# CDCgov/NowcastAutoGP

Measured on AMD Instinct MI355X. Metric: particle-logml/s (fit+forecast hot path: covariance assembly + Cholesky + logml + predictive per (particle, scenario) item), n=2048 64-particle SMC, higher is better.
Workload: dtype f64

## Files before the change

nowcastautogp_amd/csrc/ngp_api.hip:

```cpp
#include <algorithm>
#include <chrono>
#include <cmath>
#include <condition_variable>
#include <cstdio>
#include <cstdlib>
#include <cstring>
#include <dlfcn.h>
#include <map>
#include <memory>
#include <mutex>
#include <new>
#include <string>
#include <vector>

#include "ngp_internal.h"

using namespace ngp;

#define HIPCHK(expr)                                                     \
    do {                                                                 \
        hipError_t e__ = (expr);                                         \
        if (e__ != hipSuccess) return (ngp_status)(e__ > 0 ? e__ : 999); \
    } while (0)

namespace {
class PinnedPool {
    std::mutex mu;
    std::multimap<size_t, void *> free_;
    std::map<void *, std::pair<size_t, bool>> live_;
    size_t cached_ = 0;
    static constexpr size_t MAX_CACHED = (size_t)256 << 20, MAX_PINNED_BLOCK = (size_t)8 << 20;
    static size_t size_class(size_t n) {
        size_t c = 4096;
        while (c < n) c <<= 1;
        return c;
    }
public:
    void *take(size_t n) {
        const size_t c = size_class(n);
        {
            std::lock_guard<std::mutex> lk(mu);
            auto it = free_.find(c);
            if (it != free_.end()) {
                void *p = it->second;
                free_.erase(it);
                cached_ -= c;
                return p;
            }
        }
        void *p = nullptr;
        bool pinned = c <= MAX_PINNED_BLOCK &&
                      hipHostMalloc(&p, c, hipHostMallocPortable | hipHostMallocMapped) == hipSuccess && p;
        if (!pinned) {
            (void)hipGetLastError();
            p = std::malloc(c);
            if (!p) throw std::bad_alloc();
        }
        std::lock_guard<std::mutex> lk(mu);
        live_[p] = {c, pinned};
        return p;
    }
    bool is_pinned(const void *p) {
        std::lock_guard<std::mutex> lk(mu);
        auto it = live_.find(const_cast<void *>(p));
        return it != live_.end() && it->second.second;
    }
    void give(void *p) {
        std::lock_guard<std::mutex> lk(mu);
        auto it = live_.find(p);
        if (it == live_.end()) return;
        const size_t c = it->second.first;
        if (c <= MAX_PINNED_BLOCK && (c <= ((size_t)256 << 10) || cached_ + c <= MAX_CACHED)) {
            free_.emplace(c, p);
            cached_ += c;
            return;
        }
        const bool pinned = it->second.second;
        live_.erase(it);
        if (pinned) (void)hipHostFree(p);
        else std::free(p);
    }
    ~PinnedPool() {
        for (auto &kv : free_) {
// ... 552 lines not shown
    if (!c || !out) return NGP_ERR_ARG;
    std::lock_guard<std::mutex> lk(c->mu);
    *out = c->prof;
    return NGP_OK;
}

struct ngp_job {
    ngp_ctx *ctx = nullptr;
    JobGeom g{};
    int n = 0;
    bool ran = false;
    DevProgram *progs = nullptr;
    double *t0 = nullptr, *taux = nullptr, *y0 = nullptr, *ya = nullptr;
    double *logdet = nullptr, *G = nullptr, *work = nullptr, *zbuf = nullptr;
    int32_t *info = nullptr, *qpts = nullptr;
    double *logml_base = nullptr, *logml_full = nullptr, *mu = nullptr, *sigma = nullptr;
    int64_t work_stride = 0;
    std::vector<void *> owned;
    PinVec<unsigned char> h_in, h_out;
    size_t out_off[5] = {}, out_bytes = 0;
    bool zeroed = false, copy_in_flight = false;
    bool out_fetched = false;
    ngp_spec spec{};
    std::vector<int32_t> fill_chain, fill_other, fill_single;
    int32_t *fill_chain_d = nullptr, *fill_other_d = nullptr, *fill_single_d = nullptr;
    std::vector<int32_t> refine_steps;
    std::vector<double> refine_delta, frac32;
};

namespace {

struct EventTimer {
    struct Rec { int cls; hipEvent_t a, b; double flops, bytes; };
    std::vector<Rec> recs;
    bool on;
    hipStream_t s;
    EventTimer(bool on_, hipStream_t s_) : on(on_), s(s_) {}
    ~EventTimer() {
        for (auto &r : recs) {
            (void)hipEventDestroy(r.a);
            (void)hipEventDestroy(r.b);
        }
    }
    template <class F> void run(int cls, double flops, double bytes, F &&f,
                                hipStream_t on_stream = nullptr) {
        if (!on) { f(); return; }
        hipStream_t es = on_stream ? on_stream : s;
        Rec r{cls, nullptr, nullptr, flops, bytes};
        (void)hipEventCreate(&r.a);
        (void)hipEventCreate(&r.b);
        (void)hipEventRecord(r.a, es);
        f();
        (void)hipEventRecord(r.b, es);
        recs.push_back(r);
    }
    void resolve(ngp_profile &p) {
        for (auto &r : recs) {
            float ms = 0.f;
            if (hipEventElapsedTime(&ms, r.a, r.b) == hipSuccess) {
                p.ms[r.cls] += ms;
                p.launches[r.cls] += 1;
                p.flops[r.cls] += r.flops;
                p.bytes[r.cls] += r.bytes;
            }
            (void)hipEventDestroy(r.a);
            (void)hipEventDestroy(r.b);
        }
        recs.clear();
    }
};


struct Lane {
    hipStream_t main, side;
    hipEvent_t fork, join;
    ngp_ctx *ctx;
};
inline Lane lane_of(ngp_ctx *c) { return Lane{c->stream, c->side, c->ev_fork, c->ev_join, c}; }

constexpr size_t MAX_CHUNK_ITEMS = 65535;
inline bool item_too_large(int64_t item_stride) { return item_stride * 8 > (int64_t)0x7fffffff; }
constexpr int MIXED_REORDER = 16;
constexpr int AHEAD_EARLY_MAX_ITEMS = 512;
constexpr int TWO_LANE_MIN_ITEMS = 64, TWO_LANE_MIN_NB = 24;
void factor_chunk(const Lane &ln, const JobGeom &g, const ChunkPtrs &p_in, int bc, EventTimer &tm,
                  size_t dinv_step = 0, const DevSpec *sp = nullptr, int32_t *order_buf = nullptr,
                  unsigned *order_prev = nullptr, bool half = false) {
    ChunkPtrs p0 = p_in;
    const bool mixed = sp != nullptr && p0.L32 != nullptr;
    hipStream_t s = ln.main;
    SmallPlan spl;
    if (!mixed && dinv_step == 0 && small_job(g, bc, &spl)) {
        const double nn = 16.0 * spl.nbe;
        tm.run(13, bc * small_flops(g, spl), bc * 8.0 * (nn * nn * (spl.ident ? 1.5 : 1.0) + 2.0 * g.naux * nn),
               [&] { launch_chol_small(g, p0, bc, spl, s); });
        return;
    }
    if (!half && bc <= AHEAD_EARLY_MAX_ITEMS && !mixed && !g.aux_identity && g.nb0 >= 8 && !g.invariant &&
        ln.ctx->splitk_reserve(bc) == NGP_OK)
        p0.splitk_part = ln.ctx->splitk_part;
    const int nl = ngp_ctx::MAX_LANES;
    if (!half && !mixed && nl >= 2 && bc >= TWO_LANE_MIN_ITEMS && bc <= AHEAD_EARLY_MAX_ITEMS &&
        g.nb0 >= TWO_LANE_MIN_NB && ln.main == ln.ctx->stream && ln.ctx->make_lanes(nl)) {
        ngp_ctx *c = ln.ctx;
        (void)hipEventRecord(c->ev_lane_go, s);
        std::vector<EventTimer> tms;
        tms.reserve((size_t)nl);
        int h0 = 0;
        for (int i = 0; i < nl; ++i) {
            const int h1 = (int)((long)bc * (i + 1) / nl);
            ChunkPtrs pi = p0;
            pi.L += (size_t)h0 * g.item_stride;
            pi.dinv += (size_t)h0 * NB * NB;
            pi.progs += h0;
            pi.logdet += h0;
            pi.info += h0;
            if (pi.tab) pi.tab += (size_t)h0 * g.maxstat * g.R;
            pi.n_fill_single = (int32_t)((long)p0.n_fill_single * (h1 - h0) / bc);
            if (pi.splitk_part) pi.splitk_part += (size_t)h0 * SPLITK_SLOTS * 4 * 64 * 64;
            if (i == 0) {
                factor_chunk(ln, g, pi, h1 - h0, tm, dinv_step, sp, order_buf, order_prev, true);
            } else {
                const Lane li{c->lane_main[i], c->lane_side[i], c->lane_fork[i], c->lane_join[i], c};
                tms.emplace_back(tm.on, li.main);
                (void)hipStreamWaitEvent(li.main, c->ev_lane_go, 0);
                factor_chunk(li, g, pi, h1 - h0, tms.back(), dinv_step, sp, order_buf, order_prev, true);
                (void)hipEventRecord(c->lane_done[i], li.main);
            }
            h0 = h1;
        }
        for (int i = 1; i < nl; ++i) (void)hipStreamWaitEvent(s, c->lane_done[i], 0);
        for (auto &t : tms) {
            tm.recs.insert(tm.recs.end(), t.recs.begin(), t.recs.end());
            t.recs.clear();
        }
        return;
    }
    const double nrows_aux = (double)g.naux;
    const double lazy_frac =
        (g.toep && p0.n_fill_single > 0 && !mixed) ? std::min(1.0, (double)p0.n_fill_single / bc) : 0.0;
    bool ahead_pending = false;
    const int o = (g.nb0 >= 3 && (g.nb0 & 1)) ? 1 : 0;
    for (int jj = 0; jj < g.nb0; ++jj) {
        const bool fat = jj >= o && ((jj - o) % 2 == 0) && (jj + 1 < g.nb0);
        const bool thin = jj >= o && ((jj - o) % 2 == 1);
        const int mode = fat ? COL_FAT : (thin ? COL_THIN : COL_FULL);
        const int ahead = (fat && jj + 2 < g.nb0) ? 1 : 0;
        const int k0_col = thin ? (jj - 1) * NB : 0;
        const int k0_diag = thin ? (jj - 1) * NB : (jj - o >= 2 ? (jj - 2) * NB : 0);
        const double k = (double)jj * NB;
        const double kd = k - k0_diag;
        ChunkPtrs p = p0;
        p.dinv = p0.dinv + (size_t)jj * dinv_step;
        if (ahead_pending && ((jj - o) % 2 == 0)) {
            (void)hipStreamWaitEvent(s, ln.join, 0);
            ahead_pending = false;
        }
        const bool ahead_early = bc <= AHEAD_EARLY_MAX_ITEMS;
        auto launch_ahead = [&] {
            (void)hipEventRecord(ln.fork, s);
            (void)hipStreamWaitEvent(ln.side, ln.fork, 0);
            tm.run(8, bc * (double)NB * NB * k, bc * 8.0 * NB * k,
                   [&] { launch_diag_ahead(g, p0, bc, jj, ln.side); }, ln.side);
            (void)hipEventRecord(ln.join, ln.side);
            ahead_pending = true;
        };
        if (ahead && jj > 0 && ahead_early) launch_ahead();
        tm.run(1, bc * ((double)NB * NB * kd + (double)NB * NB * NB / 3.0),
               bc * 8.0 * (NB * kd + 2.0 * NB * NB),
               [&] { launch_chol_diag(g, p, bc, jj, k0_diag, s); });
        double rows = (double)(g.n0 - (jj + 1) * NB) + nrows_aux;
        const double kc = k - k0_col;
        double rows_kc = rows * kc;
        if (g.aux_identity) {
            rows = (double)(g.n0 - (jj + 1) * NB) + (double)(g.naux - g.n0);
            rows_kc = rows * kc;
            for (int a = 0; a <= jj && a < g.nb0; ++a) {
                rows += NB;
                rows_kc += NB * std::max(0.0, k - std::max((double)k0_col, (double)a * NB));
            }
        }
        double fl = 2.0 * NB * rows_kc + rows * (double)NB * NB;
        double by = 8.0 * (rows_kc + NB * kc + 2.0 * rows * NB);
        if (fat) {
            fl += 2.0 * NB * rows_kc;
            by += 8.0 * (NB * k + 2.0 * rows * NB);
        }
        if (lazy_frac > 0.0 && (fat || (mode == COL_FULL && jj == 0))) {
            const double rm = (double)(g.n0 - (jj + 1) * NB);
            by -= lazy_frac * 8.0 * NB * (rm + (fat ? std::max(0.0, rm - NB) : 0.0));
        }
        tm.run(fat ? (mixed ? 9 : (g.aux_identity ? 12 : 0)) : 6, bc * fl, bc * by,
               [&] { launch_chol_col(g, p, bc, jj, mode, k0_col, s, sp); });
        if (mixed && fat && order_buf && jj >= 8 && jj % MIXED_REORDER == 8) {
            if (launch_mixed_order(p0, order_prev, order_buf, bc, s)) p0.order = order_buf;
        }
        if (ahead && jj > 0 && !ahead_early) launch_ahead();
    }
    if (ahead_pending) {
        (void)hipStreamWaitEvent(s, ln.join, 0);
        ahead_pending = false;
    }
}

constexpr size_t STAGE_KEEP_BYTES = (size_t)4 << 20, FETCH_PACKED_BYTES = (size_t)1 << 20;

template <class T> ngp_status job_alloc(ngp_job *j, T **p, size_t count) {
    void *v = nullptr;
    ngp_status st = j->ctx->alloc(&v, count * sizeof(T));
    if (st) return st;
    j->owned.push_back(v);
    *p = (T *)v;
    return NGP_OK;
}

ngp_status stage_general(ngp_ctx *c, int P, const ngp_kernel *kernels, int n, const double *t,
                         const double *y, int64_t ldy, int d, const double *t_add, int D,
                         const double *y_add, int64_t ld_yadd_item, int m, const double *t_new,
                         int noise_on_new, ngp_job **out, const double *const *yrows = nullptr) {
    if (!c || !out || !kernels || P <= 0 || n < 0 || d < 0 || m < 0 || D <= 0) return NGP_ERR_ARG;
    if (n + d <= 0) return NGP_ERR_ARG;
    if ((n > 0 && (!t || (!y && !yrows))) || (d > 0 && (!t_add || !y_add)) || (m > 0 && !t_new))
        return NGP_ERR_ARG;
    *out = nullptr;
    auto yrow = [&](int b) { return yrows ? yrows[b] : y + (int64_t)b * ldy; };
    std::vector<DevProgram> hp((size_t)P);
    int maxstat = 0, maxcp = 0;
    for (int i = 0; i < P; ++i) {
        int ns = 0, nc = 0, nt = 0;
        ngp_status st = compile_program(&kernels[i], &hp[(size_t)i], nullptr, &ns, &nc, &nt);
        if (st) return st;
        maxstat = std::max(maxstat, nt);
        maxcp = std::max(maxcp, nc);
    }
    JobGeom g{};
    g.B = P;
    g.n0 = (n / NB) * NB;
    g.nb0 = g.n0 / NB;
    g.tail = n - g.n0;
    g.da = g.tail + d;
    g.d = d;
    g.m = m;
    g.naux = g.da + m + 1;
    if (g.naux > NGP_MAX_AUX) return NGP_ERR_TOO_LARGE;
    g.naux_pad = (g.naux + NB - 1) / NB * NB;
    g.D = D;
    g.noise_on_new = noise_on_new ? 1 : 0;
    g.y_shared = (ldy == 0 && !yrows) ? 1 : 0;
    g.ld = g.n0;
    g.item_stride = (int64_t)(g.n0 + g.naux_pad) * g.n0;
    if (item_too_large(g.item_stride)) return NGP_ERR_TOO_LARGE;
    g.npts = g.n0 + g.da + m;
    g.n_real = g.n0;
    g.aux_identity = 0;
    g.maxstat = std::max(maxstat, 1);
    g.maxcp = std::max(maxcp, 1);
    std::vector<int32_t> h_q;
    int32_t toep_stride = 0;
    if (g.n0 > 0) {
        std::vector<double> allt((size_t)g.npts);
        for (int i = 0; i < n; ++i) allt[(size_t)i] = t[i];
        for (int a = 0; a < d; ++a) allt[(size_t)(n + a)] = t_add[a];
        for (int i = 0; i < m; ++i) allt[(size_t)(n + d + i)] = t_new[i];
        double hh = 0.0;
        int R = 0;
        if (detect_lattice(allt, &hh, &h_q, &R)) {
            g.lattice = 1;
            g.h = hh;
            g.R = R;
            if (g.nb0 >= 2) {
                const long st0 = (long)h_q[1] - (long)h_q[0];
                bool reg = st0 != 0;
                for (int i = 2; i < g.n0 && reg; ++i)
                    reg = (long)h_q[(size_t)i] - (long)h_q[(size_t)i - 1] == st0;
                if (reg) toep_stride = (int32_t)std::labs(st0);
// ... 147 lines not shown
                   });
    };
    backward(0);
    std::vector<double> dprev((size_t)bc, 1.0), dboth(2 * (size_t)bc, 0.0);
    std::vector<int32_t> active((size_t)bc);
    for (int i = 0; i < bc; ++i) { steps[i] = 0; delta_out[i] = 0.0; active[(size_t)i] = i; }
    for (int it = 1;; ++it) {
        tm.run(10, na * 2.0 * naux * n0 * n0, na * 8.0 * 3.0 * naux * n0,
               [&] { launch_kapply(g, pf, rb.A, rb.X, rb.R, na, sp, s); });
        tm.run(10, na * 4.0 * naux * naux * n0, na * 8.0 * 3.0 * naux * n0, [&] {
            launch_refine_gram(g, rb.A, rb.X, rb.R, rb.S, rb.T, rb.U, Gchunk, rb.delta, na,
                               pf.items, s);
        });
        HIPCHK(hipMemcpyAsync(dboth.data(), rb.delta, sizeof(double) * 2 * (size_t)bc,
                              hipMemcpyDeviceToHost, s));
        HIPCHK(hipStreamSynchronize(s));
        std::vector<int32_t> still;
        for (int i : active) {
            const double d = dboth[2 * (size_t)i];
            double rho = dboth[2 * (size_t)i + 1];
            if (it > 1) rho = std::max(rho, d / dprev[(size_t)i]);
            const double est = d * std::min(rho, 1.0);
            steps[i] = it;
            delta_out[i] = d;
            dprev[(size_t)i] = d;
            if (!(est <= spec.refine_tol)) still.push_back(i);
        }
        active.swap(still);
        if (active.empty() || it >= spec.refine_max) break;
        na = (int)active.size();
        HIPCHK(hipMemcpy(rb.items, active.data(), 4 * (size_t)na, hipMemcpyHostToDevice));
        pf.items = rb.items;
        for (int i : active)
            HIPCHK(hipMemcpyAsync(p.L + (size_t)i * g.item_stride + (size_t)g.n0 * g.ld,
                                  rb.R + (size_t)i * g.naux_pad * g.n0,
                                  (size_t)g.naux_pad * g.n0 * 8, hipMemcpyDeviceToDevice, s));
        for (int jj = 0; jj < g.nb0; ++jj) {
            ChunkPtrs pj = pf;
            pj.dinv = p.dinv + (size_t)jj * mstep;
            tm.run(10, na * naux * (double)NB * NB, na * 8.0 * 3.0 * naux * NB,
                   [&] { launch_chol_col(g, pj, na, jj, COL_AUX, jj * NB, s); });
            tm.run(10, na * naux * 2.0 * NB * (double)(g.n0 - (jj + 1) * NB),
                   na * 8.0 * (g.n0 - (jj + 1) * NB) * (2.0 * naux + NB),
                   [&] { launch_aux_update(g, pj, na, jj, s); });
        }
        backward(1);
    }
    for (int i : active) not_refined->push_back(i);
    return NGP_OK;
}

}

extern "C" ngp_status ngp_job_run(ngp_job *j) {
    if (!j) return NGP_ERR_ARG;
    ngp_ctx *c = j->ctx;
    std::lock_guard<std::mutex> lk(c->mu);
    HIPCHK(hipSetDevice(c->device));
    const JobGeom &g = j->g;
    hipStream_t s = c->stream;
    const DevSpec sp = dev_spec(j->spec);
    EventTimer tm(c->profiling, s);
    if (!j->zeroed && !(g.n0 > 0 && small_job(g, g.B) && j->spec.precision != NGP_PREC_MIXED)) {
        HIPCHK(hipMemsetAsync(j->logdet, 0, sizeof(double) * (size_t)g.B, s));
        HIPCHK(hipMemsetAsync(j->info, 0, sizeof(int32_t) * (size_t)g.B, s));
    }
    j->zeroed = false;
    const bool mixed = j->spec.precision == NGP_PREC_MIXED && g.nb0 >= 2 && g.nb0 <= 129 &&
                       !g.aux_identity;
    const bool refine = mixed && j->spec.refine_max > 0;
    j->refine_steps.assign((size_t)g.B, 0);
    j->refine_delta.assign((size_t)g.B, 0.0);
    j->frac32.assign((size_t)g.B, 0.0);
    void *Lbuf = nullptr, *dinv = nullptr, *tab = nullptr, *sig = nullptr;
    void *L32 = nullptr, *tmx = nullptr, *cnt = nullptr, *order_buf = nullptr, *order_prev = nullptr;
    RefineBufs rb;
    bool single_chunk = false;
    if (g.n0 > 0) {
        const size_t tab_bytes = g.lattice ? sizeof(double) * (size_t)g.maxstat * g.R : 0;
        const size_t sig_bytes = g.lattice ? sizeof(double) * (size_t)g.maxcp * g.npts : 0;
        const size_t l_bytes = (size_t)g.item_stride * sizeof(double);
        const size_t nbt = (size_t)g.nb0 + (size_t)g.naux_pad / NB;
        const size_t aux_bytes = sizeof(double) * (size_t)g.naux_pad * g.n0;
        size_t item_bytes = l_bytes + tab_bytes + sig_bytes + sizeof(double) * NB * NB;
        if (mixed)
            item_bytes += l_bytes / 2 + 4 * nbt * g.nb0 + aux_bytes + 16 +
                          (refine ? sizeof(double) * NB * NB * (size_t)g.nb0 + 2 * aux_bytes +
                                        16 * (size_t)g.naux * g.naux + 8 * (size_t)g.naux + 20
                                  : 0);
        if ((size_t)g.B * item_bytes > c->mem_cap) c->refresh_mem_cap();
        const size_t bc_max = std::min<size_t>(
            std::min<size_t>((size_t)g.B, MAX_CHUNK_ITEMS), std::max<size_t>(1, c->mem_cap / item_bytes));
        size_t nchunks = ((size_t)g.B + bc_max - 1) / bc_max;
        int Bc = 0;
        size_t mstep = 0;
        ngp_status st = NGP_OK;
        auto take_all = [&](WsPlan &dalloc) -> ngp_status {
            ngp_status st = dalloc(&Lbuf, l_bytes * (size_t)Bc);
            if (!st) st = dalloc(&dinv, sizeof(double) * (size_t)Bc * NB * NB * (refine ? g.nb0 : 1));
            if (!st && g.lattice) st = dalloc(&tab, tab_bytes * (size_t)Bc);
            if (!st && g.lattice) st = dalloc(&sig, sig_bytes * (size_t)Bc);
            if (!st && mixed) {
                st = dalloc(&L32, (l_bytes / 2) * (size_t)Bc);
                if (!st) st = dalloc(&tmx, 4 * nbt * g.nb0 * (size_t)Bc);
                if (!st) st = dalloc(&cnt, 8 * (size_t)Bc);
                if (!st) st = dalloc(&order_buf, 4 * (size_t)Bc);
                if (!st) st = dalloc(&order_prev, 4 * (size_t)Bc);
                if (!st) st = dalloc((void **)&rb.X, aux_bytes * (size_t)Bc);
            }
            if (!st && refine) {
                st = dalloc((void **)&rb.A, aux_bytes * (size_t)Bc);
                if (!st) st = dalloc((void **)&rb.R, aux_bytes * (size_t)Bc);
                if (!st) st = dalloc((void **)&rb.S, 8 * (size_t)g.naux * g.naux * Bc);
                if (!st) st = dalloc((void **)&rb.T, 8 * (size_t)g.naux * g.naux * Bc);
                if (!st) st = dalloc((void **)&rb.U, 8 * (size_t)g.naux * Bc);
                if (!st) st = dalloc((void **)&rb.delta, 16 * (size_t)Bc);
                if (!st) st = dalloc((void **)&rb.items, 4 * (size_t)Bc);
            }
            return st;
        };
        for (;; nchunks *= 2) {
            Bc = (int)(((size_t)g.B + nchunks - 1) / nchunks);
            mstep = refine ? (size_t)Bc * NB * NB : 0;
            WsPlan measure{c, true}, take{c, false};
            (void)take_all(measure);
            st = c->ws_reserve(measure.total);
            if (!st) st = take_all(take);
            if (st != NGP_ERR_TOO_LARGE || Bc <= 1) break;
        }
        single_chunk = Bc >= g.B;
        if (st) return st;
        const Lane ln = lane_of(c);
        const double nrows_aux = (double)g.naux;
        for (int b0 = 0; b0 < g.B; b0 += Bc) {
            const int bc = std::min(Bc, g.B - b0);
            ChunkPtrs p{};
            p.L = (double *)Lbuf;
            p.dinv = (double *)dinv;
            p.progs = j->progs + b0;
            p.t0 = j->t0;
            p.taux = j->taux;
            p.y0 = j->y0 + (g.y_shared ? 0 : (int64_t)b0 * g.n0);
            p.logdet = j->logdet + b0;
            p.info = j->info + b0;
            p.tab = (double *)tab;
            p.sig = (double *)sig;
            p.qpts = j->qpts;
            if (j->fill_other_d) {
                auto range = [&](const std::vector<int32_t> &v, const int32_t *dev,
                                 const int32_t **ptr, int32_t *cnt) {
                    const auto lo = std::lower_bound(v.begin(), v.end(), b0);
                    const auto hi = std::lower_bound(v.begin(), v.end(), b0 + bc);
                    *ptr = dev + (lo - v.begin());
                    *cnt = (int32_t)(hi - lo);
                };
                range(j->fill_chain, j->fill_chain_d, &p.fill_chain, &p.n_fill_chain);
                range(j->fill_other, j->fill_other_d, &p.fill_other, &p.n_fill_other);
                range(j->fill_single, j->fill_single_d, &p.fill_single, &p.n_fill_single);
                p.fill_base = b0;
            }
            if (mixed) {
                p.L32 = (float *)L32;
                p.tmax = (float *)tmx;
                p.mixcnt = (unsigned *)cnt;
                p.auxX = rb.X;
                HIPCHK(hipMemsetAsync(cnt, 0, 8 * (size_t)bc, s));
            }
            if (g.lattice)
                tm.run(4, 0.0, 0.0, [&] { launch_tables(g, p, bc, sp, s); });
            const double fill_elems =
                (double)bc * ((double)g.n0 * (g.n0 + NB) / 2.0 + nrows_aux * g.n0) -
                (g.toep ? (double)p.n_fill_single * ((double)g.n0 * (g.n0 - NB) / 2.0) : 0.0);
            tm.run(4, 0.0, 8.0 * fill_elems, [&] { launch_fill(g, p, bc, sp, s); });
            if (mixed) HIPCHK(hipMemsetAsync(order_prev, 0, 4 * (size_t)bc, s));
            double *Gchunk = j->G + (int64_t)b0 * g.naux * g.naux;
            const bool gram_inside = !mixed && mstep == 0 && small_job(g, bc);
            if (gram_inside) p.G = Gchunk;
            factor_chunk(ln, g, p, bc, tm, mstep, mixed ? &sp : nullptr, (int32_t *)order_buf,
                         (unsigned *)order_prev);
            if (!gram_inside)
                tm.run(2, bc * nrows_aux * nrows_aux * g.n0, bc * 8.0 * nrows_aux * g.n0,
                       [&] { launch_gram(g, (const double *)Lbuf, Gchunk, bc, s); });
            if (mixed) {
                std::vector<unsigned> hc(2 * (size_t)bc);
                HIPCHK(hipMemcpyAsync(hc.data(), cnt, 8 * (size_t)bc, hipMemcpyDeviceToHost, s));
                std::vector<int> bad;
                if (refine) {
                    ngp_status rs = refine_chunk(c, g, p, rb, Gchunk, bc, mstep, j->spec, sp, tm,
                                                 j->refine_steps.data() + b0,
                                                 j->refine_delta.data() + b0, &bad);
                    if (rs) { tm.resolve(c->prof); return rs; }
                } else {
                    HIPCHK(hipStreamSynchronize(s));
                }
                for (int i = 0; i < bc; ++i) {
                    const double a = hc[2 * (size_t)i], b = hc[2 * (size_t)i + 1];
                    j->frac32[(size_t)(b0 + i)] = (a + b) > 0.0 ? a / (a + b) : 0.0;
                }
                if (!bad.empty()) {
                    std::vector<int32_t> hi((size_t)bc);
                    HIPCHK(hipMemcpy(hi.data(), p.info, 4 * (size_t)bc, hipMemcpyDeviceToHost));
                    for (int i : bad)
                        if (hi[(size_t)i] == 0) hi[(size_t)i] = NGP_INFO_NOT_REFINED;
                    HIPCHK(hipMemcpy(p.info, hi.data(), 4 * (size_t)bc, hipMemcpyHostToDevice));
                }
            }
        }
    }
    EpiPtrs e{};
    e.progs = j->progs;
    e.taux = j->taux;
    e.G = j->G;
    e.ya = j->ya;
    e.logdet = j->logdet;
    e.info = j->info;
    e.work = j->work;
    e.zbuf = j->zbuf;
    e.logml_base = j->logml_base;
    e.logml_full = j->logml_full;
    e.mu = j->mu;
    e.sigma = j->sigma;
// ... 1923 lines not shown
```

nowcastautogp_amd/csrc/ngp_col_kernels.h:

```cpp
#pragma once
#include <algorithm>

#include "ngp_mfma.h"

namespace ngp {

struct NoProbe {
    __device__ __forceinline__ void mark(int) {}
    template <class T>
    __device__ __forceinline__ void mark_after(int, T) {}
    __device__ __forceinline__ void drain() {}
    __device__ __forceinline__ void emit_diag(int, int, int) {}
    __device__ __forceinline__ void emit_col(int, int, int, int, int, int, bool) {}
    __device__ __forceinline__ void begin(int, int, int) {}
    __device__ __forceinline__ void sweep(int) {}
};

__device__ __forceinline__ void sqrt_and_rcp(double a, double &d, double &r) {
    double y = __builtin_amdgcn_rsq(a);
    const double h = 0.5 * a;
    y = y * fma(-h * y, y, 1.5);
    y = y * fma(-h * y, y, 1.5);
    d = a * y;
    d = fma(fma(-d, d, a), 0.5 * y, d);
    r = fma(fma(-d, y, 1.0), y, y);
}

__device__ __forceinline__ int tri(int r, int c) { return ((r * (r + 1)) >> 1) + c; }
constexpr int TRI = NB * (NB + 1) / 2;

template <class Probe = NoProbe>
__global__ __launch_bounds__(256, 4) void chol_diag_kernel(JobGeom g, ChunkPtrs p, int j, int k0) {
    __shared__ double Mt[TRI];
    __shared__ double Lt[TRI];
    __shared__ double pan[NB][4];
    __shared__ double dblk[16];
    __shared__ double dinvd[4];
    __shared__ double rdg[NB];
    __shared__ double logs[NB];
    __shared__ double Ts[TB][TB + 1];
    __shared__ int bad;
    const int item = blockIdx.x;
    const int tid = threadIdx.x, lane = tid & 63;
    const int wave = __builtin_amdgcn_readfirstlane(tid >> 6);
    const long ld = g.ld;
    double *Lit = p.L + (long)item * g.item_stride;
    double *Lj = Lit + (long)j * NB * ld;
    const int kmax = j * NB;
    const int r16 = lane & 15, q = lane >> 4;
    const int wr = wave >> 1, wc = wave & 1;
    Probe probe;
    probe.mark_after(0, lane);

    if (tid == 0) bad = 0;

    if (!(wr == 0 && wc == 1)) {
        double acc4[2][2][4];
#pragma unroll
        for (int a = 0; a < 2; ++a)
#pragma unroll
            for (int b = 0; b < 2; ++b)
#pragma unroll
                for (int r = 0; r < 4; ++r) acc4[a][b][r] = 0.0;
        const double *pa = Lj + (long)(32 * wr + r16) * ld + 2 * q;
        const double *pb = Lj + (long)(32 * wc + r16) * ld + 2 * q;
        double kt[2][2][4];
#pragma unroll
        for (int mt = 0; mt < 2; ++mt)
#pragma unroll
            for (int nt = 0; nt < 2; ++nt)
#pragma unroll
                for (int s = 0; s < 4; ++s)
                    kt[mt][nt][s] = Lj[(long)(32 * wr + 16 * mt + q + 4 * s) * ld + kmax +
                                       32 * wc + 16 * nt + r16];
        for (int kc = k0; kc < kmax; kc += 16) {
            double a[2][4], b[2][4];
#pragma unroll
            for (int u = 0; u < 2; ++u) {
                const f64x2 alo = *reinterpret_cast<const f64x2 *>(pa + (long)u * 16 * ld + kc);
                const f64x2 ahi = *reinterpret_cast<const f64x2 *>(pa + (long)u * 16 * ld + kc + 8);
                const f64x2 blo = *reinterpret_cast<const f64x2 *>(pb + (long)u * 16 * ld + kc);
                const f64x2 bhi = *reinterpret_cast<const f64x2 *>(pb + (long)u * 16 * ld + kc + 8);
                a[u][0] = alo.x; a[u][1] = alo.y; a[u][2] = ahi.x; a[u][3] = ahi.y;
                b[u][0] = blo.x; b[u][1] = blo.y; b[u][2] = bhi.x; b[u][3] = bhi.y;
            }
#pragma unroll
            for (int s = 0; s < 4; ++s)
#pragma unroll
                for (int nt = 0; nt < 2; ++nt) {
                    const Rot4 br = rot4(b[nt][s]);
#pragma unroll
                    for (int mt = 0; mt < 2; ++mt) mfma16_as_4(acc4[mt][nt], a[mt][s], br);
                }
        }
        f64x4 acc[2][2];
#pragma unroll
        for (int a = 0; a < 2; ++a)
#pragma unroll
            for (int b = 0; b < 2; ++b) acc[a][b] = to_d16(acc4[a][b]);
#pragma unroll
        for (int mt = 0; mt < 2; ++mt)
#pragma unroll
            for (int nt = 0; nt < 2; ++nt)
#pragma unroll
                for (int s = 0; s < 4; ++s) {
                    const int M = 32 * wr + 16 * mt + q + 4 * s, N = 32 * wc + 16 * nt + r16;
                    if (M >= N) Mt[tri(M, N)] = kt[mt][nt][s] - acc[mt][nt][s];
                }
    }
    __syncthreads();
    probe.mark_after(1, lane);

    const int bi = tid >> 4, bj = tid & 15;
    {
        double a[4][4];
#pragma unroll
        for (int r = 0; r < 4; ++r)
#pragma unroll
            for (int c = 0; c < 4; ++c) {
                const int R = 4 * bi + r, C = 4 * bj + c;
                a[r][c] = (R >= C) ? Mt[tri(R, C)] : 0.0;
            }
        for (int kb = 0; kb < NB / 4; ++kb) {
            if (bi == kb && bj == kb) {
                double dks[4];
#pragma unroll
                for (int kc = 0; kc < 4; ++kc) {
                    const double akk = a[kc][kc];
                    double dk, inv;
                    sqrt_and_rcp(akk, dk, inv);
                    if (!(akk > 0.0) && bad == 0) bad = 4 * kb + kc + 1;
                    dks[kc] = dk;
                    dinvd[kc] = inv;
                    rdg[4 * kb + kc] = inv;
// ... 39 lines not shown
            __syncthreads();
            if (bj > kb && bi >= bj) {
                double li[4][4], lj[4][4];
#pragma unroll
                for (int r = 0; r < 4; ++r)
#pragma unroll
                    for (int pp = 0; pp < 4; ++pp) {
                        li[r][pp] = pan[4 * bi + r][pp];
                        lj[r][pp] = pan[4 * bj + r][pp];
                    }
#pragma unroll
                for (int pp = 0; pp < 4; ++pp)
#pragma unroll
                    for (int r = 0; r < 4; ++r)
#pragma unroll
                        for (int c = 0; c < 4; ++c) a[r][c] -= li[r][pp] * lj[c][pp];
            }
        }
#pragma unroll
        for (int r = 0; r < 4; ++r) {
            const int R = 4 * bi + r;
            f64x2 lo, hi;
            lo.x = (R >= 4 * bj) ? a[r][0] : 0.0;
            lo.y = (R >= 4 * bj + 1) ? a[r][1] : 0.0;
            hi.x = (R >= 4 * bj + 2) ? a[r][2] : 0.0;
            hi.y = (R >= 4 * bj + 3) ? a[r][3] : 0.0;
            double *dst = Lj + (long)R * ld + kmax + 4 * bj;
            *reinterpret_cast<f64x2 *>(dst) = lo;
            *reinterpret_cast<f64x2 *>(dst + 2) = hi;
#pragma unroll
            for (int c = 0; c < 4; ++c)
                if (R >= 4 * bj + c) Lt[tri(R, 4 * bj + c)] = a[r][c];
        }
    }
    __syncthreads();
    probe.mark_after(2, lane);
    if (tid < NB) logs[tid] = log(Lt[tri(tid, tid)]);

    if (tid < NB) {
        const int b = tid >> 4, c = tid & 15;
        double x[TB];
#pragma unroll
        for (int i = 0; i < TB; ++i) {
            double sum = (i == c) ? 1.0 : 0.0;
            int off = tri(TB * b + i, TB * b);
            if (i > 0) asm volatile("" : "+v"(off) : "v"(x[i - 1]));
            const double *lrow = &Lt[off];
#pragma unroll
            for (int pp = 0; pp < i; ++pp) sum -= lrow[pp] * x[pp];
            x[i] = sum * rdg[TB * b + i];
        }
#pragma unroll
        for (int i = 0; i < TB; ++i)
            if (i >= c) Mt[tri(TB * b + i, TB * b + c)] = x[i];
    }
    __syncthreads();
    probe.mark_after(3, lane);
    {
        const int ra = tid >> 4, cb = tid & 15;
        for (int dist = 1; dist < NB / TB; ++dist)
            for (int ct = dist; ct < NB / TB; ++ct) {
                const int jt = ct - dist;
                double t = 0.0;
                for (int kt = jt; kt < ct; ++kt)
#pragma unroll
                    for (int pp = 0; pp < TB; ++pp) {
                        const double mv = Mt[tri(TB * kt + pp, TB * jt + cb)];
                        t += Lt[tri(TB * ct + ra, TB * kt + pp)] * ((kt > jt || pp >= cb) ? mv : 0.0);
                    }
                Ts[ra][cb] = t;
                __syncthreads();
                double mv = 0.0;
#pragma unroll
                for (int pp = 0; pp < TB; ++pp) {
                    const double md = Mt[tri(TB * ct + ra, TB * ct + pp)];
                    mv -= ((pp <= ra) ? md : 0.0) * Ts[pp][cb];
                }
                Mt[tri(TB * ct + ra, TB * jt + cb)] = mv;
                __syncthreads();
            }
    }
    probe.mark_after(4, lane);
    {
        double *dv = p.dinv + (long)item * (NB * NB);
        for (int e = tid; e < NB * NB; e += 256) {
            const int strip = e >> 6, l = e & 63;
            const int cb4 = strip >> 2, jt = strip & 3;
            const int R = 4 * cb4 + (l & 3), C = 16 * jt + 4 * ((l >> 2) & 3) + (l >> 4);
            dv[e] = (R >= C) ? Mt[tri(R, C)] : 0.0;
        }
    }
    if (tid == 0) {
        double s = 0.0;
        for (int k = 0; k < NB; ++k) s += logs[k];
        p.logdet[item] += s;
        if (bad && p.info[item] == 0) p.info[item] = kmax + bad;
    }
    probe.mark_after(5, lane);
    probe.emit_diag(j, tid, item);
}

template <int NF>
struct Frag8 {
    f64x2 v[NF];
};
template <int NF>
__device__ __forceinline__ void load_frag8(Frag8<NF> &f, const double *p, long ld) {
#pragma unroll
    for (int u = 0; u < NF; ++u) f.v[u] = *reinterpret_cast<const f64x2 *>(p + (long)u * 16 * ld);
}
template <int NA>
__device__ __forceinline__ void mfma_frag8(double (&acc)[NA][4][4], const Frag8<NA> &a,
                                           const Frag8<4> &b) {
#pragma unroll
    for (int it = 0; it < 4; ++it) {
        const Rot4 br = rot4(b.v[it].x);
#pragma unroll
        for (int jt = 0; jt < NA; ++jt) mfma16_as_4(acc[jt][it], a.v[jt].x, br);
    }
#pragma unroll
    for (int it = 0; it < 4; ++it) {
        const Rot4 br = rot4(b.v[it].y);
#pragma unroll
        for (int jt = 0; jt < NA; ++jt) mfma16_as_4(acc[jt][it], a.v[jt].y, br);
    }
}

template <int NA>
__device__ __forceinline__ void gemm_rows(double (&acc)[NA][4][4], const double *pa,
                                          const double *pb, long ld, int k0, int k1) {
    if (k1 <= k0) return;
    Frag8<NA> a0, a1;
    Frag8<4> b0, b1;
    load_frag8(a0, pa + k0, ld);
    load_frag8(b0, pb + k0, ld);
    for (int kc = k0; kc < k1; kc += 16) {
        load_frag8(a1, pa + kc + 8, ld);
        load_frag8(b1, pb + kc + 8, ld);
        mfma_frag8(acc, a0, b0);
        if (kc + 16 < k1) {
            load_frag8(a0, pa + kc + 16, ld);
            load_frag8(b0, pb + kc + 16, ld);
        }
        mfma_frag8(acc, a1, b1);
    }
}

constexpr int EPI_PITCH = 66;
constexpr int EPI_M_BYTES = NB * NB * 8;
constexpr int EPI_WAVE_BYTES = 16 * EPI_PITCH * 8;
constexpr int EPI_LDS_BYTES = EPI_M_BYTES + 4 * EPI_WAVE_BYTES;

__device__ __forceinline__ void stage_mstrips(double *lds_m, const double *mstrips, int tid) {
#pragma unroll
    for (int i = 0; i < 8; ++i) {
        const int idx = tid + 256 * i;
        reinterpret_cast<f64x2 *>(lds_m)[idx] = reinterpret_cast<const f64x2 *>(mstrips)[idx];
    }
}

template <bool SHADOW = false, bool SYNTH = false, class Probe = NoProbe, bool KROWS = false>
__device__ __forceinline__ void solve_and_store_lds(const double (*acc4)[4][4], double *Lr,
                                                    const double *lds_m, long ld, int kmax,
                                                    int lane, double *buf, Probe &probe,
                                                    float *Lr32 = nullptr,
                                                    float *tmax_out = nullptr, int synth = 0,
                                                    const double *ksl = nullptr, int nit = 4) {
    double amax = 0.0;
    const int n16 = lane & 15, isub = lane >> 4;
    const int jj0 = 4 * (n16 >> 2) + isub;
    const double *ksl0 = ksl ? ksl + 15 - jj0 : nullptr;
    f64x2 kvr[8];
    double kvp[4][4];
    const int hrow = lane >> 5, c2 = 2 * (lane & 31);
    bool from_rows = KROWS && ksl0 == nullptr;
    if constexpr (SYNTH) from_rows = from_rows && synth == 0;
    auto k_elems = [&](int it, double (&kv)[4][4]) {
        if (ksl0) {
#pragma unroll
            for (int jt = 0; jt < 4; ++jt)
#pragma unroll
                for (int r = 0; r < 4; ++r)
// ... 752 lines not shown
#pragma unroll
                for (int jl = 0; jl < 2; ++jl)
#pragma unroll
                    for (int it = 0; it < 4; ++it)
#pragma unroll
                        for (int r = 0; r < 4; ++r)
                            acc4[2 * a + jl][it][r] =
                                t64[(16 * jl + jj0) * P64 + 16 * it + ((r16 + 4 * r) & 15)];
                __syncthreads();
            }
        }
        if (n64 > 0) {
            unsigned long long lo = m64lo, hi = m64hi;
            const int nch = 4 * n64;
            int kt_cur = pop(lo, hi), sub = 1;
            stage(0, kt_cur * NB);
            __syncthreads();
            for (int c = 0; c < nch; ++c) {
                const int cur = c & 1;
                if (c + 1 < nch) {
                    if (sub == 4) {
                        kt_cur = pop(lo, hi);
                        sub = 0;
                    }
                    stage(cur ^ 1, kt_cur * NB + LDS_KC * sub);
                    ++sub;
                }
                mult_chunk_pipelined<2 * BLKB>(acc4, smem + cur * STAGE, a_addr, b_addr);
                __syncthreads();
            }
        }
    }
    if constexpr (SPLITK == 1) {
        double *mine = p.splitk_part +
                       ((((long)slot * SPLITK_SLOTS + (long)grp * st.splits + piece) * 4 + wave) *
                        (64 * 64)) + lane;
#pragma unroll
        for (int jt = 0; jt < 4; ++jt)
#pragma unroll
            for (int it = 0; it < 4; ++it)
#pragma unroll
                for (int r = 0; r < 4; ++r) mine[((jt * 4 + it) * 4 + r) * 64] = acc4[jt][it][r];
        return;
    }
    if constexpr (SPLITK == 2) {
        const double *part = p.splitk_part +
                             ((((long)slot * SPLITK_SLOTS + (long)grp * st.splits) * 4 + wave) *
                              (64 * 64)) + lane;
#pragma unroll
        for (int jt = 0; jt < 4; ++jt)
#pragma unroll
            for (int it = 0; it < 4; ++it)
#pragma unroll
                for (int r = 0; r < 4; ++r) acc4[jt][it][r] = part[((jt * 4 + it) * 4 + r) * 64];
        for (int q2 = 1; q2 < st.splits; ++q2) {
            const double *pq = part + (long)q2 * 4 * (64 * 64);
            double v[4][4][4];
#pragma unroll
            for (int jt = 0; jt < 4; ++jt)
#pragma unroll
                for (int it = 0; it < 4; ++it)
#pragma unroll
                    for (int r = 0; r < 4; ++r) v[jt][it][r] = pq[((jt * 4 + it) * 4 + r) * 64];
#pragma unroll
            for (int jt = 0; jt < 4; ++jt)
#pragma unroll
                for (int it = 0; it < 4; ++it)
#pragma unroll
                    for (int r = 0; r < 4; ++r) acc4[jt][it][r] += v[jt][it][r];
        }
    }
    static_assert(EPI_LDS_BYTES + TOEP_LDS_BYTES <= 2 * STAGE,
                  "epilogue LDS must fit the stage buffers");
    probe.mark(3);
    const double *ksl = nullptr;
    if (structured) {
        double *sl = reinterpret_cast<double *>(smem + EPI_LDS_BYTES) + wave * 128;
        struct_slice(sl, g, p, item, (int)tile_row0(tile), col ? kmax + NB : kmax, lane);
        ksl = sl;
    }
    stage_mstrips(reinterpret_cast<double *>(smem), p.dinv + (long)item * (NB * NB), tid);
    __syncthreads();
    probe.mark(4);
    if (!valid) return;

    double *Lr = Lit + tile_row0(tile) * ld;
    if (col) {
        subtract_in_place_rows(Lr, ld, (j + 1) * NB, acc4, lane,
                               reinterpret_cast<double *>(smem + EPI_M_BYTES + wave * EPI_WAVE_BYTES),
                               IDENT && synth != 0, ksl, nit);
    } else if constexpr (MIXED) {
        const int rt = (tile < st.nmain) ? j + 1 + tile : g.nb0 + (tile - st.nmain);
        solve_and_store_lds<true>(
            acc4, Lr, reinterpret_cast<const double *>(smem), ld, kmax, lane,
            reinterpret_cast<double *>(smem + EPI_M_BYTES + wave * EPI_WAVE_BYTES), probe,
            p.L32 + (long)item * g.item_stride + tile_row0(tile) * ld,
            p.tmax + (long)item * (g.nb0 + g.naux_pad / NB) * g.nb0 + tmax_index(g, rt, j));
    } else {
        solve_and_store_lds<false, IDENT>(
            acc4, Lr, reinterpret_cast<const double *>(smem), ld, kmax, lane,
            reinterpret_cast<double *>(smem + EPI_M_BYTES + wave * EPI_WAVE_BYTES), probe, nullptr,
            nullptr, synth, ksl, nit);
    }
    probe.mark(5);
    probe.drain();
    probe.mark(6);
    probe.emit_col(j, lane, wg, wave, item, tile, false);
}

template <class Probe>
void launch_chol_diag_t(const JobGeom &g, const ChunkPtrs &p, int Bc, int j, int k0, hipStream_t s) {
    hipLaunchKernelGGL(chol_diag_kernel<Probe>, dim3(Bc), dim3(256), 0, s, g, p, j, k0);
}

template <class Probe>
void launch_chol_col_t(const JobGeom &g, const ChunkPtrs &p, int Bc, int j, int mode, int k0,
                     hipStream_t s, const DevSpec *sp) {
    ColStep st{};
    const bool mixed = p.L32 != nullptr && sp != nullptr;
    if (mixed) {
        st.c32 = sp->mixed_tau / (64.0 * 5.9604644775390625e-08);
        st.jitter = sp->jitter;
    }
    st.j = j;
    st.k0 = k0;
    st.nmain = (mode == COL_AUX) ? 0 : g.nb0 - 1 - j;
    st.ntiles = st.nmain + g.naux_pad / NB;
    if (st.ntiles <= 0) return;
    const int bpad = (Bc + 7) / 8 * 8;
    const dim3 blk(256);
    st.first_touch = (mode == COL_FAT || (mode == COL_FULL && k0 == 0 && j == 0)) ? 1 : 0;
    if (mode == COL_FAT) {
        st.groups = (st.ntiles + 1) / 2;
        const dim3 grid(st.groups * bpad);
        int splits = 1;
        if (!mixed && !g.aux_identity && p.splitk_part) {
            const int nchunks = j * NB / LDS_KC;
            splits = std::min(std::min(8, SPLITK_SLOTS / std::max(st.groups, 1)),
                              std::min(nchunks / 8, 384 / std::max(st.groups * Bc, 1)));
        }
        st.splits = std::max(splits, 1);
        if (splits >= 2) {
            hipLaunchKernelGGL((chol_col_glds_kernel<false, Probe, false, 1>),
                               dim3(st.groups * splits * bpad), blk, 0, s, g, p, Bc, st);
            hipLaunchKernelGGL((chol_col_glds_kernel<false, Probe, false, 2>), grid, blk, 0, s, g, p,
                               Bc, st);
        } else if (mixed)
            hipLaunchKernelGGL((chol_col_glds_kernel<true, Probe>), grid, blk, 0, s, g, p, Bc, st);
        else if (g.aux_identity)
            hipLaunchKernelGGL((chol_col_glds_kernel<false, Probe, true>), grid, blk, 0, s, g, p, Bc, st);
        else
            hipLaunchKernelGGL((chol_col_glds_kernel<false, Probe>), grid, blk, 0, s, g, p, Bc, st);
    } else if (mode == COL_THIN && k0 == j * NB - NB && j > 0) {
        st.groups = (st.ntiles + 3) / 4;
        const dim3 grid(st.groups * bpad);
        if (mixed)
            hipLaunchKernelGGL((chol_col_thin_kernel<true, Probe>), grid, blk, 0, s, g, p, Bc, st);
        else if (g.aux_identity)
            hipLaunchKernelGGL((chol_col_thin_kernel<false, Probe, true>), grid, blk, 0, s, g, p, Bc, st);
        else
            hipLaunchKernelGGL((chol_col_thin_kernel<false, Probe>), grid, blk, 0, s, g, p, Bc, st);
    } else {
        st.groups = (st.ntiles + 3) / 4;
        const dim3 grid(st.groups * bpad);
        if (mixed)
            hipLaunchKernelGGL(chol_col_kernel<true>, grid, blk, 0, s, g, p, Bc, st);
        else if (g.aux_identity)
            hipLaunchKernelGGL((chol_col_kernel<false, true>), grid, blk, 0, s, g, p, Bc, st);
        else if (g.toep && st.first_touch)
            hipLaunchKernelGGL((chol_col_kernel<false, false, true>), grid, blk, 0, s, g, p, Bc, st);
        else
            hipLaunchKernelGGL(chol_col_kernel<false>, grid, blk, 0, s, g, p, Bc, st);
    }
}

}
```

nowcastautogp_amd/csrc/ngp_internal.h:

```cpp
#pragma once
#include <hip/hip_runtime.h>
#include <stdint.h>

#include <algorithm>

#include "../../include/ngp.h"

namespace ngp {

constexpr int NB = 64;
constexpr int TB = 16;
constexpr int DEV_STACK = 8;
constexpr int SPLITK_SLOTS = 16;

constexpr int OP_CP_SWAPPED = 9;
constexpr int OP_TABLE = 10;
constexpr int RLEAF_TABLE = 1, RLEAF_LINEAR = 2;
constexpr int MAX_TABLES = NGP_MAX_OPS / 2;

struct DevProgram {
    int32_t n_ops;
    int32_t n_params;
    double  noise;
    uint8_t ops[NGP_MAX_OPS];
    uint8_t slot[NGP_MAX_OPS];
    uint8_t first[NGP_MAX_OPS];
    uint8_t poff[NGP_MAX_OPS];
    double  params[NGP_MAX_PARAMS];
    int32_t n_rops, n_tab;
    int32_t rchain, rpad_;
    uint8_t rops[NGP_MAX_OPS];
    uint8_t rslot[NGP_MAX_OPS];
    uint8_t rpoff[NGP_MAX_OPS];
    uint8_t rleaf[NGP_MAX_OPS];
    uint8_t tb_first[MAX_TABLES];
    uint8_t tb_last[MAX_TABLES];
};
static_assert(sizeof(DevProgram) % 8 == 0, "DevProgram is copied as 8-byte words");
__host__ __device__ inline bool prog_single_table(const DevProgram *P) {
    return P->n_rops == 1 && P->rops[0] == OP_TABLE;
}
__host__ __device__ inline int prog_structure(const DevProgram *P) {
    return (P->n_rops == 1 && P->rops[0] == OP_TABLE) ? 1 : 0;
}
struct DevSpec {
    int32_t se_form, periodic_form, cp_form, precision;
    double  jitter;
    double  mixed_tau;
};

struct JobGeom {
    int32_t B;
    int32_t n0;
    int32_t nb0;
    int32_t da;
    int32_t tail;
    int32_t m;
    int32_t naux;
    int32_t naux_pad;
    int32_t D;
    int32_t d;
    int32_t noise_on_new;
    int32_t y_shared;
    int32_t lattice;
    int32_t R;
    int32_t npts;
    int32_t maxstat;
    int32_t maxcp;
    int32_t n_real;
    int32_t aux_identity;
    int32_t maxops;
    int32_t aux_e1;
    int32_t toep;
    int32_t tab_sub;
    int32_t invariant;
    int32_t short_series;
    int32_t pad_;
    double  h;
    int64_t ld;
    int64_t item_stride;
};

struct ChunkPtrs {
    double       *L;
    double       *dinv;
    const DevProgram *progs;
    const DevProgram *progs_src;
    const double *t0;
    const double *taux;
    const double *y0;
    double       *logdet;
    int32_t      *info;
    double       *tab;
    double       *sig;
    const int32_t *qpts;
    double       *dtab;
    float        *L32;
    float        *tmax;
    unsigned     *mixcnt;
    double       *auxX;
    const int32_t *order;
    const int32_t *fill_chain, *fill_other, *fill_single;
    int32_t n_fill_chain, n_fill_other, n_fill_single, fill_base;
    double       *G;
    const int32_t *items;
    double       *splitk_part;
};

struct EpiPtrs {
    const DevProgram *progs;
    const double *taux;
    const double *G;
    const double *ya;
    const double *logdet;
    int32_t      *info;
    double       *work;
    double       *zbuf;
    double       *logml_base;
    double       *logml_full;
    double       *mu;
    double       *sigma;
    int64_t       work_stride;
    const double *tab, *sig;
    const int32_t *qpts;
};

constexpr int SM_WAVES = 8, SM_THREADS = 64 * SM_WAVES;
constexpr int SM_NSLOT = 20;
constexpr int SM_DSTR = 17;
constexpr int SM_MAX_PANEL = 34;
constexpr int SM_MAX_SWEEPS = 4;
constexpr int SM_MAX_ITEMS = 4096;

struct SmallSweep {
    int32_t main;
    int32_t i0, i1, a0, a1;
};
struct SmallPlan {
    int32_t nbe;
    int32_t nsweeps;
    int32_t ident;
    int32_t npanel;
    uint64_t colwave;
    SmallSweep sw[SM_MAX_SWEEPS];
};

constexpr int SM_LDS_FIXED = 8 * (16 * 256 + 16 * 16 * SM_DSTR + 256 + 32);
inline int small_lds_bytes(const SmallPlan &pl) { return SM_LDS_FIXED + pl.npanel * 2048; }

inline bool small_plan(const JobGeom &g, SmallPlan *pl) {
    if (g.n0 <= 0 || g.nb0 > 4 || g.aux_e1 || g.toep) return false;
    const int nb16 = g.n0 / 16, nbe = (g.n_real + 15) / 16;
    if (nbe < 1 || nbe > nb16) return false;
    const int cap_main = (SM_WAVES - 1) * SM_NSLOT, cap_aux = SM_WAVES * SM_NSLOT;
    SmallPlan p{};
    p.nbe = nbe;
    p.ident = g.aux_identity ? 1 : 0;
    int used = nbe * (nbe - 1) / 2;
    if (used > cap_main) return false;
    int ns = 0, npanel = nbe;
    if (g.aux_identity) {
        const int ytile = nb16;
        if (used + nbe > cap_main) return false;
        p.sw[ns++] = SmallSweep{1, 0, 0, ytile, ytile + 1};
        p.sw[ns++] = SmallSweep{2, 0, nbe, 0, 0};
        npanel = std::max(npanel, nbe + 1);
        int load[SM_WAVES] = {};
        for (int j = 0; j < nbe; ++j) {
            int best = 0;
            for (int w = 1; w < SM_WAVES; ++w) {
                const int sb = load[best % 4] + load[best % 4 + 4], sw_ = load[w % 4] + load[w % 4 + 4];
                if (sw_ < sb || (sw_ == sb && load[w] < load[best])) best = w;
            }
            load[best] += (nbe - j) * (nbe - j - 1) / 2 + 1;
            p.colwave |= (uint64_t)best << (4 * j);
        }
    } else {
        const int nba = (g.naux + 15) / 16;
        int a = std::min(nba, (cap_main - used) / nbe);
        a = std::min(a, SM_MAX_PANEL - nbe);
        p.sw[ns++] = SmallSweep{1, 0, 0, 0, a};
        npanel = std::max(npanel, nbe + a);
        while (a < nba) {
            if (ns == SM_MAX_SWEEPS) return false;
            const int b = std::min(nba, a + std::min(cap_aux / nbe, SM_MAX_PANEL - nbe));
            p.sw[ns++] = SmallSweep{0, 0, 0, a, b};
            npanel = std::max(npanel, nbe + b - a);
            a = b;
        }
// ... 81 lines not shown
```

Measured before the change: 17220.

## Fuse next-column diagonal Cholesky into fat column kernel for large batches

For batches larger than the ahead-early threshold, the fat column kernel's group-0 workgroup now factors the next diagonal block (j+1) after finishing its tile, reusing the stage LDS. The separate chol_diag launch for the following thin column is skipped. A second dinv slot is allocated so the next block's inverse does not overwrite the one still being read. This removes one kernel launch and one sync point per column pair, but serialises the diagonal factorization onto the tail of one workgroup per item and adds LDS aliasing and extra workspace.

```diff
diff --git a/nowcastautogp_amd/csrc/ngp_api.hip b/nowcastautogp_amd/csrc/ngp_api.hip
--- a/nowcastautogp_amd/csrc/ngp_api.hip
+++ b/nowcastautogp_amd/csrc/ngp_api.hip
@@ -1,4 +1,5 @@
 #include <algorithm>
+#include <atomic>
 #include <chrono>
 #include <cmath>
 #include <condition_variable>
@@ -717,6 +718,8 @@
 inline bool item_too_large(int64_t item_stride) { return item_stride * 8 > (int64_t)0x7fffffff; }
 constexpr int MIXED_REORDER = 16;
 constexpr int AHEAD_EARLY_MAX_ITEMS = 512;
+static std::atomic<int> g_diag_fuse{1};
+extern "C" void ngp_debug_set_diag_fuse(int on) { g_diag_fuse.store(on); }
 constexpr int TWO_LANE_MIN_ITEMS = 64, TWO_LANE_MIN_NB = 24;
 void factor_chunk(const Lane &ln, const JobGeom &g, const ChunkPtrs &p_in, int bc, EventTimer &tm,
                   size_t dinv_step = 0, const DevSpec *sp = nullptr, int32_t *order_buf = nullptr,
@@ -753,6 +756,7 @@
             if (pi.tab) pi.tab += (size_t)h0 * g.maxstat * g.R;
             pi.n_fill_single = (int32_t)((long)p0.n_fill_single * (h1 - h0) / bc);
             if (pi.splitk_part) pi.splitk_part += (size_t)h0 * SPLITK_SLOTS * 4 * 64 * 64;
+            if (pi.dinv2) pi.dinv2 += (size_t)h0 * NB * NB;
             if (i == 0) {
                 factor_chunk(ln, g, pi, h1 - h0, tm, dinv_step, sp, order_buf, order_prev, true);
             } else {
@@ -775,6 +779,8 @@
     const double lazy_frac =
         (g.toep && p0.n_fill_single > 0 && !mixed) ? std::min(1.0, (double)p0.n_fill_single / bc) : 0.0;
     bool ahead_pending = false;
+    const bool fuse_diag = g_diag_fuse.load(std::memory_order_relaxed) && bc > AHEAD_EARLY_MAX_ITEMS &&
+                           !mixed && !g.aux_identity && !p0.splitk_part && (dinv_step != 0 || p0.dinv2);
     const int o = (g.nb0 >= 3 && (g.nb0 & 1)) ? 1 : 0;
     for (int jj = 0; jj < g.nb0; ++jj) {
         const bool fat = jj >= o && ((jj - o) % 2 == 0) && (jj + 1 < g.nb0);
@@ -787,6 +793,9 @@
         const double kd = k - k0_diag;
         ChunkPtrs p = p0;
         p.dinv = p0.dinv + (size_t)jj * dinv_step;
+        const bool diag_done = fuse_diag && thin;
+        if (diag_done && !dinv_step) p.dinv = p0.dinv2;
+        if (fuse_diag && fat) p.dinv_next = dinv_step ? p0.dinv + (size_t)(jj + 1) * dinv_step : p0.dinv2;
         if (ahead_pending && ((jj - o) % 2 == 0)) {
             (void)hipStreamWaitEvent(s, ln.join, 0);
             ahead_pending = false;
@@ -801,9 +810,10 @@
             ahead_pending = true;
         };
         if (ahead && jj > 0 && ahead_early) launch_ahead();
-        tm.run(1, bc * ((double)NB * NB * kd + (double)NB * NB * NB / 3.0),
-               bc * 8.0 * (NB * kd + 2.0 * NB * NB),
-               [&] { launch_chol_diag(g, p, bc, jj, k0_diag, s); });
+        auto diag_fl = [&](double kd_) { return bc * ((double)NB * NB * kd_ + (double)NB * NB * NB / 3.0); };
+        auto diag_by = [&](double kd_) { return bc * 8.0 * (NB * kd_ + 2.0 * NB * NB); };
+        if (!diag_done)
+            tm.run(1, diag_fl(kd), diag_by(kd), [&] { launch_chol_diag(g, p, bc, jj, k0_diag, s); });
         double rows = (double)(g.n0 - (jj + 1) * NB) + nrows_aux;
         const double kc = k - k0_col;
         double rows_kc = rows * kc;
@@ -825,7 +835,12 @@
             const double rm = (double)(g.n0 - (jj + 1) * NB);
             by -= lazy_frac * 8.0 * NB * (rm + (fat ? std::max(0.0, rm - NB) : 0.0));
         }
-        tm.run(fat ? (mixed ? 9 : (g.aux_identity ? 12 : 0)) : 6, bc * fl, bc * by,
+        double fl_all = bc * fl, by_all = bc * by;
+        if (fuse_diag && fat) {
+            fl_all += diag_fl(NB);
+            by_all += diag_by(NB);
+        }
+        tm.run(fat ? (mixed ? 9 : (g.aux_identity ? 12 : 0)) : 6, fl_all, by_all,
                [&] { launch_chol_col(g, p, bc, jj, mode, k0_col, s, sp); });
         if (mixed && fat && order_buf && jj >= 8 && jj % MIXED_REORDER == 8) {
             if (launch_mixed_order(p0, order_prev, order_buf, bc, s)) p0.order = order_buf;
@@ -1139,7 +1154,8 @@
         const size_t l_bytes = (size_t)g.item_stride * sizeof(double);
         const size_t nbt = (size_t)g.nb0 + (size_t)g.naux_pad / NB;
         const size_t aux_bytes = sizeof(double) * (size_t)g.naux_pad * g.n0;
-        size_t item_bytes = l_bytes + tab_bytes + sig_bytes + sizeof(double) * NB * NB;
+        const size_t mslots = refine ? (size_t)g.nb0 : (mixed ? 1 : 2);
+        size_t item_bytes = l_bytes + tab_bytes + sig_bytes + sizeof(double) * NB * NB * (refine ? 1 : mslots);
         if (mixed)
             item_bytes += l_bytes / 2 + 4 * nbt * g.nb0 + aux_bytes + 16 +
                           (refine ? sizeof(double) * NB * NB * (size_t)g.nb0 + 2 * aux_bytes +
@@ -1154,7 +1170,7 @@
         ngp_status st = NGP_OK;
         auto take_all = [&](WsPlan &dalloc) -> ngp_status {
             ngp_status st = dalloc(&Lbuf, l_bytes * (size_t)Bc);
-            if (!st) st = dalloc(&dinv, sizeof(double) * (size_t)Bc * NB * NB * (refine ? g.nb0 : 1));
+            if (!st) st = dalloc(&dinv, sizeof(double) * (size_t)Bc * NB * NB * mslots);
             if (!st && g.lattice) st = dalloc(&tab, tab_bytes * (size_t)Bc);
             if (!st && g.lattice) st = dalloc(&sig, sig_bytes * (size_t)Bc);
             if (!st && mixed) {
@@ -1194,6 +1210,7 @@
             ChunkPtrs p{};
             p.L = (double *)Lbuf;
             p.dinv = (double *)dinv;
+            if (mslots == 2) p.dinv2 = (double *)dinv + (size_t)Bc * NB * NB;
             p.progs = j->progs + b0;
             p.t0 = j->t0;
             p.taux = j->taux;
diff --git a/nowcastautogp_amd/csrc/ngp_col_kernels.h b/nowcastautogp_amd/csrc/ngp_col_kernels.h
--- a/nowcastautogp_amd/csrc/ngp_col_kernels.h
+++ b/nowcastautogp_amd/csrc/ngp_col_kernels.h
@@ -29,18 +29,30 @@
 __device__ __forceinline__ int tri(int r, int c) { return ((r * (r + 1)) >> 1) + c; }
 constexpr int TRI = NB * (NB + 1) / 2;
 
-template <class Probe = NoProbe>
-__global__ __launch_bounds__(256, 4) void chol_diag_kernel(JobGeom g, ChunkPtrs p, int j, int k0) {
-    __shared__ double Mt[TRI];
-    __shared__ double Lt[TRI];
-    __shared__ double pan[NB][4];
-    __shared__ double dblk[16];
-    __shared__ double dinvd[4];
-    __shared__ double rdg[NB];
-    __shared__ double logs[NB];
-    __shared__ double Ts[TB][TB + 1];
-    __shared__ int bad;
-    const int item = blockIdx.x;
+struct DiagLds {
+    double Mt[TRI];
+    double Lt[TRI];
+    double pan[NB][4];
+    double dblk[16];
+    double dinvd[4];
+    double rdg[NB];
+    double logs[NB];
+    double Ts[TB][TB + 1];
+    int bad;
+};
+
+template <class Probe>
+__device__ __forceinline__ void chol_diag_block(const JobGeom &g, const ChunkPtrs &p, int item, int j,
+                                                int k0, double *dv, DiagLds &sh, Probe &probe) {
+    double(&Mt)[TRI] = sh.Mt;
+    double(&Lt)[TRI] = sh.Lt;
+    double(&pan)[NB][4] = sh.pan;
+    double(&dblk)[16] = sh.dblk;
+    double(&dinvd)[4] = sh.dinvd;
+    double(&rdg)[NB] = sh.rdg;
+    double(&logs)[NB] = sh.logs;
+    double(&Ts)[TB][TB + 1] = sh.Ts;
+    int &bad = sh.bad;
     const int tid = threadIdx.x, lane = tid & 63;
     const int wave = __builtin_amdgcn_readfirstlane(tid >> 6);
     const long ld = g.ld;
@@ -49,7 +61,6 @@
     const int kmax = j * NB;
     const int r16 = lane & 15, q = lane >> 4;
     const int wr = wave >> 1, wc = wave & 1;
-    Probe probe;
     probe.mark_after(0, lane);
 
     if (tid == 0) bad = 0;
@@ -255,7 +266,7 @@
     }
     probe.mark_after(4, lane);
     {
-        double *dv = p.dinv + (long)item * (NB * NB);
+        dv += (long)item * (NB * NB);
         for (int e = tid; e < NB * NB; e += 256) {
             const int strip = e >> 6, l = e & 63;
             const int cb4 = strip >> 2, jt = strip & 3;
@@ -270,7 +281,14 @@
         if (bad && p.info[item] == 0) p.info[item] = kmax + bad;
     }
     probe.mark_after(5, lane);
-    probe.emit_diag(j, tid, item);
+}
+
+template <class Probe = NoProbe>
+__global__ __launch_bounds__(256, 4) void chol_diag_kernel(JobGeom g, ChunkPtrs p, int j, int k0) {
+    __shared__ DiagLds sh;
+    Probe probe;
+    chol_diag_block(g, p, (int)blockIdx.x, j, k0, p.dinv, sh, probe);
+    probe.emit_diag(j, threadIdx.x, blockIdx.x);
 }
 
 template <int NF>
@@ -1189,10 +1207,13 @@
     stage_mstrips(reinterpret_cast<double *>(smem), p.dinv + (long)item * (NB * NB), tid);
     __syncthreads();
     probe.mark(4);
-    if (!valid) return;
+    bool fuse_diag = false;
+    if constexpr (!MIXED && !IDENT && SPLITK == 0) fuse_diag = p.dinv_next != nullptr && grp == 0;
+    if (!valid && !fuse_diag) return;
 
     double *Lr = Lit + tile_row0(tile) * ld;
-    if (col) {
+    if (!valid) {
+    } else if (col) {
         subtract_in_place_rows(Lr, ld, (j + 1) * NB, acc4, lane,
                                reinterpret_cast<double *>(smem + EPI_M_BYTES + wave * EPI_WAVE_BYTES),
                                IDENT && synth != 0, ksl, nit);
@@ -1213,6 +1234,14 @@
     probe.drain();
     probe.mark(6);
     probe.emit_col(j, lane, wg, wave, item, tile, false);
+    if constexpr (!MIXED && !IDENT && SPLITK == 0) {
+        static_assert(sizeof(DiagLds) <= 2 * STAGE, "chol_diag's LDS must fit the stage buffers");
+        if (fuse_diag) {
+            __syncthreads();
+            NoProbe np;
+            chol_diag_block(g, p, item, j + 1, kmax, p.dinv_next, *reinterpret_cast<DiagLds *>(smem), np);
+        }
+    }
 }
 
 template <class Probe>
diff --git a/nowcastautogp_amd/csrc/ngp_internal.h b/nowcastautogp_amd/csrc/ngp_internal.h
--- a/nowcastautogp_amd/csrc/ngp_internal.h
+++ b/nowcastautogp_amd/csrc/ngp_internal.h
@@ -105,6 +105,8 @@
     double       *G;
     const int32_t *items;
     double       *splitk_part;
+    double       *dinv_next;
+    double       *dinv2;
 };
 
 struct EpiPtrs {
```

After: 16700 (median of 2 runs). 0.97x the previous value.
